# researchaccelerator-hub/distributed-crawler

Hardware: AMD Instinct MI355X
Metric: posts/sec (whole node) synthetic feed (higher is better)
Workload: dtype uint8; 1 GPU; model=telegram-crawl 1k-channels x 10k-posts per GPU (BASELINE config #2, weak-scaled), global_batch=1250000, seq_len=0, platform=telegram, parallelism=dp1, channels_per_gpu=1000, posts_per_channel=10000, chunk_posts=1250000, new_discoveries=998486, sink=pinned, pinned=True, max_comments_per_post=3

## Files before the change

### crawler_amd/ops/csrc/common.h

```cpp
#pragma once

#include <hip/hip_runtime.h>
#include <stdint.h>

#define WAVE 64
#define DEV __device__ __forceinline__

typedef unsigned int __attribute__((aligned(1))) u32_unal;
#ifndef CRAWL_NT_STORES
#define CRAWL_NT_STORES 0
#endif
DEV void nt_store_u32(unsigned char* p, unsigned v) {
#if CRAWL_NT_STORES
  __builtin_nontemporal_store(v, (u32_unal*)p);
#else
  __builtin_memcpy(p, &v, 4);
#endif
}
DEV void nt_store_u8(unsigned char* p, unsigned char v) {
#if CRAWL_NT_STORES
  __builtin_nontemporal_store(v, p);
#else
  *p = v;
#endif
}

namespace crawl {

DEV int lane_id() { return threadIdx.x & (WAVE - 1); }
DEV int wave_id() { return threadIdx.x >> 6; }


DEV bool is_ascii_letter(uint8_t c) {
  return (c >= 'a' && c <= 'z') || (c >= 'A' && c <= 'Z');
}
DEV bool is_word_char(uint8_t c) {
  return is_ascii_letter(c) || (c >= '0' && c <= '9') || c == '_';
}
DEV uint8_t to_lower(uint8_t c) {
  return (c >= 'A' && c <= 'Z') ? (c + 32) : c;
}

DEV int u16_units_of_byte(uint8_t b) {
  if (b < 0x80) return 1;
  if (b < 0xC0) return 0;
  if (b < 0xF0) return 1;
  return 2;
}

__device__ const uint8_t ESC_CLS[256] = {
    0x06, 0x06, 0x06, 0x06, 0x06, 0x06, 0x06, 0x06, 0x06, 0x02, 0x02, 0x06, 0x06, 0x02, 0x06, 0x06,
    0x06, 0x06, 0x06, 0x06, 0x06, 0x06, 0x06, 0x06, 0x06, 0x06, 0x06, 0x06, 0x06, 0x06, 0x06, 0x06,
    0x01, 0x01, 0x02, 0x01, 0x01, 0x01, 0x06, 0x01, 0x01, 0x01, 0x01, 0x01, 0x01, 0x01, 0x01, 0x01,
    0x01, 0x01, 0x01, 0x01, 0x01, 0x01, 0x01, 0x01, 0x01, 0x01, 0x01, 0x01, 0x06, 0x01, 0x06, 0x01,
    0x01, 0x01, 0x01, 0x01, 0x01, 0x01, 0x01, 0x01, 0x01, 0x01, 0x01, 0x01, 0x01, 0x01, 0x01, 0x01,
    0x01, 0x01, 0x01, 0x01, 0x01, 0x01, 0x01, 0x01, 0x01, 0x01, 0x01, 0x01, 0x02, 0x01, 0x01, 0x01,
    0x01, 0x01, 0x01, 0x01, 0x01, 0x01, 0x01, 0x01, 0x01, 0x01, 0x01, 0x01, 0x01, 0x01, 0x01, 0x01,
    0x01, 0x01, 0x01, 0x01, 0x01, 0x01, 0x01, 0x01, 0x01, 0x01, 0x01, 0x01, 0x01, 0x01, 0x01, 0x01,
    0xFF, 0x01, 0x01, 0x01, 0x01, 0x01, 0x01, 0x01, 0x01, 0x01, 0x01, 0x01, 0x01, 0x01, 0x01, 0x01,
    0x01, 0x01, 0x01, 0x01, 0x01, 0x01, 0x01, 0x01, 0x01, 0x01, 0x01, 0x01, 0x01, 0x01, 0x01, 0x01,
    0x01, 0x01, 0x01, 0x01, 0x01, 0x01, 0x01, 0x01, 0xFF, 0xFF, 0x01, 0x01, 0x01, 0x01, 0x01, 0x01,
    0x01, 0x01, 0x01, 0x01, 0x01, 0x01, 0x01, 0x01, 0x01, 0x01, 0x01, 0x01, 0x01, 0x01, 0x01, 0x01,
    0x01, 0x01, 0x01, 0x01, 0x01, 0x01, 0x01, 0x01, 0x01, 0x01, 0x01, 0x01, 0x01, 0x01, 0x01, 0x01,
    0x01, 0x01, 0x01, 0x01, 0x01, 0x01, 0x01, 0x01, 0x01, 0x01, 0x01, 0x01, 0x01, 0x01, 0x01, 0x01,
    0x01, 0x01, 0xFF, 0x01, 0x01, 0x01, 0x01, 0x01, 0x01, 0x01, 0x01, 0x01, 0x01, 0x01, 0x01, 0x01,
    0x01, 0x01, 0x01, 0x01, 0x01, 0x01, 0x01, 0x01, 0x01, 0x01, 0x01, 0x01, 0x01, 0x01, 0x01, 0x01,
};

DEV int escape_len_at(const uint8_t* s, int n, int p) {
  uint8_t c = s[p];
  uint8_t v = ESC_CLS[c];
  if (v != 0xFF) return v;
  if (c == 0xE2) {
    if (p + 2 < n && s[p + 1] == 0x80 &&
        (s[p + 2] == 0xA8 || s[p + 2] == 0xA9))
      return 6;
    return 1;
  }
  if (c == 0x80) {
    if (p >= 1 && s[p - 1] == 0xE2 && p + 1 < n &&
        (s[p + 1] == 0xA8 || s[p + 1] == 0xA9))
      return 0;
    return 1;
  }
  if (p >= 2 && s[p - 2] == 0xE2 && s[p - 1] == 0x80) return 0;
  return 1;
}

DEV const char* HEXD() { return "0123456789abcdef"; }

DEV int escape_write_at(const uint8_t* s, int n, int p, uint8_t* out) {
  uint8_t c = s[p];
  switch (c) {
    case '"':  out[0] = '\\'; out[1] = '"';  return 2;
    case '\\': out[0] = '\\'; out[1] = '\\'; return 2;
    case '\n': out[0] = '\\'; out[1] = 'n';  return 2;
    case '\r': out[0] = '\\'; out[1] = 'r';  return 2;
    case '\t': out[0] = '\\'; out[1] = 't';  return 2;
    default: break;
  }
  if (c < 0x20 || c == '<' || c == '>' || c == '&') {
    out[0] = '\\'; out[1] = 'u'; out[2] = '0'; out[3] = '0';
    out[4] = HEXD()[c >> 4]; out[5] = HEXD()[c & 15];
    return 6;
  }
  if (c == 0xE2 && p + 2 < n && s[p + 1] == 0x80 &&
      (s[p + 2] == 0xA8 || s[p + 2] == 0xA9)) {
    out[0] = '\\'; out[1] = 'u'; out[2] = '2'; out[3] = '0'; out[4] = '2';
    out[5] = (s[p + 2] == 0xA8) ? '8' : '9';
    return 6;
  }
  if (escape_len_at(s, n, p) == 0) return 0;
  out[0] = c;
  return 1;
}


DEV int wave_prefix_excl(int v) {
  int lane = lane_id();
  for (int d = 1; d < WAVE; d <<= 1) {
    int up = __shfl_up(v, d);
    if (lane >= d) v += up;
  }
  return __shfl_up(v, 1) * (lane > 0 ? 1 : 0);
}

DEV int wave_sum(int v) {
  for (int d = WAVE / 2; d > 0; d >>= 1) v += __shfl_down(v, d);
  return __shfl(v, 0);
}


DEV int u64_dec_len(uint64_t v) {
  if (v < 10ULL) return 1;
  if (v < 100ULL) return 2;
  if (v < 1000ULL) return 3;
  if (v < 10000ULL) return 4;
  if (v < 100000ULL) return 5;
  if (v < 1000000ULL) return 6;
  if (v < 10000000ULL) return 7;
  if (v < 100000000ULL) return 8;
  if (v < 1000000000ULL) return 9;
  if (v < 10000000000ULL) return 10;
  if (v < 100000000000ULL) return 11;
  if (v < 1000000000000ULL) return 12;
  if (v < 10000000000000ULL) return 13;
  if (v < 100000000000000ULL) return 14;
  if (v < 1000000000000000ULL) return 15;
  if (v < 10000000000000000ULL) return 16;
  if (v < 100000000000000000ULL) return 17;
  if (v < 1000000000000000000ULL) return 18;
  if (v < 10000000000000000000ULL) return 19;
  return 20;
}
DEV int i64_dec_len(int64_t v) {
  return (v < 0) ? 1 + u64_dec_len((uint64_t)(-v)) : u64_dec_len((uint64_t)v);
}

DEV void rfc3339_write(uint8_t* out, int cur, long long secs) {
  long long days = secs / 86400;
  long long rem = secs % 86400;
  if (rem < 0) { rem += 86400; days -= 1; }
  int hh = (int)(rem / 3600), mm = (int)((rem % 3600) / 60),
      ss = (int)(rem % 60);
  long long z = days + 719468;
  long long era = (z >= 0 ? z : z - 146096) / 146097;
  long long doe = z - era * 146097;
  long long yoe = (doe - doe / 1460 + doe / 36524 - doe / 146096) / 365;
  long long y = yoe + era * 400;
  long long doy = doe - (365 * yoe + yoe / 4 - yoe / 100);
  long long mp = (5 * doy + 2) / 153;
  long long d = doy - (153 * mp + 2) / 5 + 1;
  long long m = mp + (mp < 10 ? 3 : -9);
  y += (m <= 2);
  int yy = (int)y, mo = (int)m, dd = (int)d;
  auto pk = [](int a, int b, int c, int e) {
    return (unsigned)a | ((unsigned)b << 8) | ((unsigned)c << 16) |
           ((unsigned)e << 24);
  };
  unsigned w0 = pk('0' + (yy / 1000) % 10, '0' + (yy / 100) % 10,
                   '0' + (yy / 10) % 10, '0' + yy % 10);
  unsigned w1 = pk('-', '0' + mo / 10, '0' + mo % 10, '-');
  unsigned w2 = pk('0' + dd / 10, '0' + dd % 10, 'T', '0' + hh / 10);
  unsigned w3 = pk('0' + hh % 10, ':', '0' + mm / 10, '0' + mm % 10);
  unsigned w4 = pk(':', '0' + ss / 10, '0' + ss % 10, 'Z');
  int lane = lane_id();
  if (lane < 5) {
    unsigned v = w0;
    if (lane == 1) v = w1;
    else if (lane == 2) v = w2;
    else if (lane == 3) v = w3;
    else if (lane == 4) v = w4;
    nt_store_u32(out + cur + 4 * lane, v);
  }
}

#define LIT(e, s)                                              \
  do {                                                         \
    if ((int)sizeof(s) - 1 <= 4)                               \
      (e).template lit_small<(int)sizeof(s) - 1>(s);           \
    else                                                       \
      (e).raw((const unsigned char*)(s), (int)sizeof(s) - 1);  \
  } while (0)

template <bool W>
struct JsonEmit {
  uint8_t* out;
  int cur;
  const uint8_t* lds;

  DEV void lds_lit(int off, int n) {
    if (W) {
      const uint8_t* s = lds + off;
      int lane = lane_id();
      int nw = n >> 2;
      for (int k = lane; k < nw; k += WAVE) {
        unsigned w;
        __builtin_memcpy(&w, s + 4 * k, 4);
        nt_store_u32(out + cur + 4 * k, w);
      }
      for (int j = (nw << 2) + lane; j < n; j += WAVE)
        nt_store_u8(out + cur + j, s[j]);
    }
    cur += n;
  }

  template <int N, int M>
  DEV void lit_small(const char (&str)[M]) {
    if (W && lane_id() == 0) {
      if (N == 1) {
        out[cur] = (unsigned char)str[0];
      } else if (N == 2) {
        unsigned short v = (unsigned short)((unsigned char)str[0] |
                                            ((unsigned char)str[1] << 8));
        __builtin_memcpy(out + cur, &v, 2);
      } else {
        unsigned v = (unsigned)(unsigned char)str[0] |
                     ((unsigned)(unsigned char)str[1] << 8) |
                     ((N > 2 ? (unsigned)(unsigned char)str[2] : 0u) << 16) |
                     ((N > 3 ? (unsigned)(unsigned char)str[3] : 0u) << 24);
        if (N == 4)
          __builtin_memcpy(out + cur, &v, 4);
        else {
          __builtin_memcpy(out + cur, &v, 2);
          out[cur + 2] = (unsigned char)str[2];
        }
      }
    }
    cur += N;
  }

  DEV void raw(const uint8_t* s, int n) {
    if (W) {
      int lane = lane_id();
      int nw = n >> 2;
      for (int k = lane; k < nw; k += WAVE) {
        unsigned w;
        __builtin_memcpy(&w, s + 4 * k, 4);
        nt_store_u32(out + cur + 4 * k, w);
      }
      for (int j = (nw << 2) + lane; j < n; j += WAVE)
        nt_store_u8(out + cur + j, s[j]);
    }
    cur += n;
  }

  static DEV bool swar_special(unsigned w) {
    unsigned hz;
    unsigned nonascii = w & 0x80808080u;
    unsigned lt20 = (w - 0x20202020u) & ~w & 0x80808080u;
    if (lt20) return true;
    hz = ((w ^ 0x22222222u) - 0x01010101u) & ~(w ^ 0x22222222u);
    hz |= ((w ^ 0x5C5C5C5Cu) - 0x01010101u) & ~(w ^ 0x5C5C5C5Cu);
    hz |= ((w ^ 0x3C3C3C3Cu) - 0x01010101u) & ~(w ^ 0x3C3C3C3Cu);
    hz |= ((w ^ 0x3E3E3E3Eu) - 0x01010101u) & ~(w ^ 0x3E3E3E3Eu);
    hz |= ((w ^ 0x26262626u) - 0x01010101u) & ~(w ^ 0x26262626u);
    if (hz & 0x80808080u) return true;
    if (nonascii) {
      unsigned e2 = ((w ^ 0xE2E2E2E2u) - 0x01010101u) & ~(w ^ 0xE2E2E2E2u);
      if (e2 & 0x80808080u) return true;
    }
    return false;
  }

  DEV void esc(const uint8_t* s, int n) {
    int lane = lane_id();
    int start = 0;
    while (start < n) {
      if (start + 4 * WAVE <= n) {
        bool risk = (start >= 1 && s[start - 1] == 0xE2) ||
                    (start >= 2 && s[start - 2] == 0xE2 &&
                     s[start - 1] == 0x80);
        if (!risk) {
          unsigned w;
          __builtin_memcpy(&w, s + start + 4 * lane, 4);
          if (__ballot(swar_special(w)) == 0) {
            if (W)
              nt_store_u32(out + cur + 4 * lane, w);
            cur += 4 * WAVE;
            start += 4 * WAVE;
            continue;
          }
        }
      }
      esc_stripe(s, n, start, lane);
      start += WAVE;
    }
  }

  DEV void esc_stripe(const uint8_t* s, int n, int start, int lane) {
    {
      int p = start + lane;
      int span = n - start;
      if (span > WAVE) span = WAVE;
      int el = (p < n) ? escape_len_at(s, n, p) : 0;
      unsigned long long dirty = __ballot(p < n && el != 1);
      if (dirty == 0) {
        if (W && p < n) nt_store_u8(out + cur + p - start, s[p]);
        cur += span;
        return;
      }
      if (W) {
        int off = wave_prefix_excl(el);
        if (p < n && el > 0) {
          escape_write_at(s, n, p, out + cur + off);
        }
      }
      cur += wave_sum(el);
    }
  }

  DEV void u64(unsigned long long v) {
    static const unsigned long long POW10[20] = {
        1ULL, 10ULL, 100ULL, 1000ULL, 10000ULL, 100000ULL, 1000000ULL,
        10000000ULL, 100000000ULL, 1000000000ULL, 10000000000ULL,
        100000000000ULL, 1000000000000ULL, 10000000000000ULL,
        100000000000000ULL, 1000000000000000ULL, 10000000000000000ULL,
        100000000000000000ULL, 1000000000000000000ULL,
        10000000000000000000ULL};
    int n = u64_dec_len(v);
    if (W) {
      int lane = lane_id();
      if (lane < n) {
        unsigned d;
        if (v <= 0xFFFFFFFFULL)
          d = ((unsigned)v / (unsigned)POW10[lane]) % 10u;
        else
          d = (unsigned)((v / POW10[lane]) % 10ULL);
        nt_store_u8(out + cur + n - 1 - lane, (uint8_t)('0' + d));
      }
    }
    cur += n;
  }
  DEV void i64(long long v) {
    if (v < 0) { LIT(*this, "-"); u64((unsigned long long)(-v)); }
    else u64((unsigned long long)v);
  }

  DEV void rfc3339(long long secs) {
    if (W) rfc3339_write(out, cur, secs);
    cur += 20;
  }
};

DEV uint64_t fnv1a64(const uint8_t* s, int n) {
  uint64_t h = 1469598103934665603ULL;
  for (int i = 0; i < n; ++i) {
    h ^= s[i];
    h *= 1099511628211ULL;
  }
  return h;
}

}
```

### crawler_amd/ops/csrc/parse_encode.hip

```cpp

#include "common.h"
#include "tg_lits.h"

namespace crawl {

#define MAX_LINKS 8
#define TG_STAGE_BYTES 3968

struct BatchView {
  const long* __restrict__ chat_id;
  const long* __restrict__ msg_id;
  const long* __restrict__ text_off;
  const int* __restrict__ date;
  const int* __restrict__ content_type;
  const int* __restrict__ views;
  const int* __restrict__ forwards;
  const int* __restrict__ media_album_id;
  const int* __restrict__ channel_idx;
  const int* __restrict__ flags;
  const int* __restrict__ text_len;
  const int* __restrict__ aux_off;
  const int* __restrict__ aux_len;
  const int* __restrict__ ent_off;
  const int* __restrict__ ent_cnt;
  const int* __restrict__ react_off;
  const int* __restrict__ react_cnt;
  const int* __restrict__ com_off;
  const int* __restrict__ com_cnt;
  const int* __restrict__ poster_off;
  const int* __restrict__ poster_len;
  const unsigned char* __restrict__ pool;
  const int* __restrict__ entities;
  const int* __restrict__ react_emoji;
  const int* __restrict__ react_count;
  const int* __restrict__ com_text_off;
  const int* __restrict__ com_text_len;
  const int* __restrict__ com_handle_off;
  const int* __restrict__ com_handle_len;
  const int* __restrict__ com_views;
  const int* __restrict__ com_replies;
  const int* __restrict__ com_react_off;
  const int* __restrict__ com_react_cnt;
  const long* __restrict__ ch_chat_id;
  const int* __restrict__ ch_member;
  const int* __restrict__ ch_postcount;
  const int* __restrict__ ch_totalviews;
  const int* __restrict__ ch_user_off;
  const int* __restrict__ ch_user_len;
  const int* __restrict__ ch_title_off;
  const int* __restrict__ ch_title_len;
  const unsigned char* __restrict__ emoji_pool;
  const int* __restrict__ emoji_off;
  const int* __restrict__ emoji_len;
  const unsigned char* __restrict__ created_str;
  int created_len;
  const unsigned char* __restrict__ capture_str;
  int capture_len;
  int n;
  int skip_media;
  long min_post_date;
  const unsigned char* __restrict__ ctname_pool;
  const int* __restrict__ ctname_off;
  const int* __restrict__ ctname_len;
};

struct LinkOut {
  unsigned char* __restrict__ name;
  unsigned char* __restrict__ name_len;
  unsigned char* __restrict__ src;
  int* __restrict__ cnt;
  unsigned long long* __restrict__ hash;
};


DEV void utf16_to_bytes(const unsigned char* s, int n, int off16, int len16,
                        int* out_start, int* out_end) {
  int lane = lane_id();
  int run = 0;
  int start = -1, end = -1;
  const int t1 = off16, t2 = off16 + len16;
  for (int base = 0; base < n; base += WAVE) {
    int p = base + lane;
    int u = (p < n) ? u16_units_of_byte(s[p]) : 0;
    int pre = run + wave_prefix_excl(u);
    bool boundary = (p < n) && u > 0;
    unsigned long long m1 = __ballot(boundary && pre == t1);
    unsigned long long m2 = __ballot(boundary && pre == t2);
    if (start < 0 && m1) start = base + __ffsll(m1) - 1;
    if (end < 0 && m2) end = base + __ffsll(m2) - 1;
    run += wave_sum(u);
    if (end >= 0) break;
  }
  if (start < 0) { *out_start = 0; *out_end = 0; return; }
  *out_start = start;
  *out_end = (end >= 0) ? end : n;
}


DEV bool is_reserved_path(const unsigned char* name, int n) {
  const char* tbl[10] = {"joinchat", "addlist", "addstickers", "addtheme",
                         "setlanguage", "share", "proxy", "socks", "login",
                         "confirm"};
  const int lens[10] = {8, 7, 11, 8, 11, 5, 5, 5, 5, 7};
  for (int k = 0; k < 10; ++k) {
    if (lens[k] != n) continue;
    bool eq = true;
    for (int j = 0; j < n; ++j) eq &= (name[j] == (unsigned char)tbl[k][j]);
    if (eq) return true;
  }
  return false;
}

DEV int match_name_at(const unsigned char* s, int hi, int q,
                      unsigned char* name, bool* reserved) {
  *reserved = false;
  if (q >= hi || !is_ascii_letter(s[q])) return 0;
  int len = 0;
  while (len < 32 && q + len < hi && is_word_char(s[q + len])) ++len;
  if (len < 5) return 0;
  for (int j = 0; j < len; ++j) name[j] = to_lower(s[q + j]);
  *reserved = is_reserved_path(name, len);
  return len;
}

DEV int find_tme(const unsigned char* s, int from, int hi, int lane) {
  for (int base = from; base + 5 <= hi; base += WAVE) {
    int p = base + lane;
    bool m = (p + 5 <= hi) && s[p] == 't' && s[p + 1] == '.' &&
             s[p + 2] == 'm' && s[p + 3] == 'e' && s[p + 4] == '/';
    unsigned long long bal = __ballot(m);
    if (bal) return base + __ffsll(bal) - 1;
  }
  return -1;
}

DEV int find_username(const unsigned char* s, int lo, int hi, int lane,
                      unsigned char* name) {
  for (int base = lo; base < hi; base += WAVE) {
    int p = base + lane;
    bool m = false;
    if (p < hi && p + 5 <= hi && is_ascii_letter(s[p])) {
      m = is_word_char(s[p + 1]) && is_word_char(s[p + 2]) &&
          is_word_char(s[p + 3]) && is_word_char(s[p + 4]);
    }
    unsigned long long bal = __ballot(m);
    if (bal) {
      int q = base + __ffsll(bal) - 1;
      int len = 0;
      while (len < 32 && q + len < hi && is_word_char(s[q + len])) ++len;
      for (int j = 0; j < len; ++j) name[j] = to_lower(s[q + j]);
      return len;
    }
  }
  return 0;
}

struct LinkList {
  unsigned char* names;
  unsigned char* lens;
  unsigned char* srcs;
  unsigned long long* hashes;
  int cnt;

  DEV void add(const unsigned char* name, int len, int src, int lane) {
    for (int k = 0; k < cnt; ++k) {
      if (lens[k] != (unsigned char)len) continue;
      bool eq = true;
      for (int j = 0; j < len; ++j) eq &= (names[k * 32 + j] == name[j]);
      if (eq) return;
    }
    if (cnt >= MAX_LINKS) return;
    if (lane == 0) {
      for (int j = 0; j < len; ++j) names[cnt * 32 + j] = name[j];
      lens[cnt] = (unsigned char)len;
      srcs[cnt] = (unsigned char)src;
      hashes[cnt] = fnv1a64(name, len);
    }
    ++cnt;
  }
};

DEV void extract_links(const BatchView& B, int i, LinkList& L, int lane) {
  int ct = B.content_type[i];
  if (ct > 6) return;
  const unsigned char* text = B.pool + B.text_off[i];
  const int tn = B.text_len[i];
  unsigned char name[32];

  const int e0 = B.ent_off[i], ec = B.ent_cnt[i];
  for (int e = e0; e < e0 + ec; ++e) {
    const int* row = B.entities + (long)e * 5;
    int etype = row[0];
    if (etype == 1) {
      const unsigned char* url = B.pool + row[3];
      int un = row[4];
      for (int from = 0;;) {
        int p = find_tme(url, from, un, lane);
        if (p < 0) break;
        bool rsv;
        int len = match_name_at(url, un, p + 5, name, &rsv);
        if (len) {
          if (!rsv) L.add(name, len, 1, lane);
          break;
        }
        from = p + 1;
      }
    } else {
      int lo, hi;
      utf16_to_bytes(text, tn, row[1], row[2], &lo, &hi);
      if (!(lo < hi && hi <= tn)) continue;
      if (etype == 0) {
        int len = find_username(text, lo, hi, lane, name);
        if (len) L.add(name, len, 0, lane);
      } else {
        for (int from = lo;;) {
          int p = find_tme(text, from, hi, lane);
          if (p < 0) break;
          bool rsv;
          int len = match_name_at(text, hi, p + 5, name, &rsv);
          if (len) {
            if (!rsv) L.add(name, len, 2, lane);
            break;
          }
          from = p + 1;
        }
      }
    }
  }

  int cursor = 0;
  int from = 0;
  while (true) {
    int p = find_tme(text, from, tn, lane);
    if (p < 0) break;
    from = p + 1;
    if (p < cursor) continue;
    bool rsv;
    int len = match_name_at(text, tn, p + 5, name, &rsv);
    if (len) {
      if (!rsv) L.add(name, len, 3, lane);
      cursor = p + 5 + len;
      from = cursor;
    }
  }
}


template <bool W>
struct Emit : JsonEmit<W> {
  DEV void qesc(const unsigned char* s, int n) {
    LIT(*this, "\"");
    this->esc(s, n);
    LIT(*this, "\"");
  }
};

struct StagedTabs {
  const unsigned char* emoji_pool;
  const int* emoji_off;
  const int* emoji_len;
  const unsigned char* created;
  const unsigned char* capture;
  const unsigned char* ctname_pool;
  const int* ctname_off;
  const int* ctname_len;
};

template <bool W, bool STAGED>
DEV int emit_line(const BatchView& B, int i, unsigned char* out,
                  LinkList& L, const unsigned char* lds_lits,
                  unsigned char* lds_stage, const StagedTabs* T) {
  const int lane = lane_id();
  Emit<W> e{};
  e.out = out;
  e.cur = 0;
  e.lds = lds_lits;
  const int c = B.channel_idx[i];
  const unsigned char* user = B.pool + B.ch_user_off[c];
  const int user_n = B.ch_user_len[c];
  const unsigned char* title = B.pool + B.ch_title_off[c];
  const int title_n = B.ch_title_len[c];
  const long pub_id = B.msg_id[i] >> 20;
  const int ct = B.content_type[i];
  const int ncom = B.com_cnt[i];
  const bool has_user = user_n > 0;
  const long chat_id_v = B.chat_id[i];
  const int media_album = B.media_album_id[i];
  const int date_v = B.date[i];
  const int views_v = B.views[i];
  const int forwards_v = B.forwards[i];
  const int ch_member_v = B.ch_member[c];
  const int ch_postcount_v = B.ch_postcount[c];
  const int ch_totalviews_v = B.ch_totalviews[c];
  const int flags_v = B.flags[i];
  const int com0_v = B.com_off[i];
  const int react0_v = B.react_off[i];
  const int reactc_v = B.react_cnt[i];
  const int poster_off_v = B.poster_off[i];
  const int poster_len_v = B.poster_len[i];
  const int text_off_v = B.text_off[i];
  const int text_len_v = B.text_len[i];
  const int aux_off_v = B.aux_off[i];
  const int aux_len_v = B.aux_len[i];
  const int ctname_off_v = B.ctname_off[ct];
  const int ctname_len_v = B.ctname_len[ct];
  const unsigned char* desc_p;
  int desc_n;
  if (ct == 0 || ct == 1 || ct == 2 || ct == 4 || ct == 14) {
    desc_p = B.pool + text_off_v;
    desc_n = text_len_v;
  } else if (ct == 3 || ct == 9 || ct == 10 || ct == 11) {
    desc_p = B.pool + aux_off_v;
    desc_n = aux_len_v;
  } else {
    desc_p = nullptr;
    desc_n = 0;
  }
  const unsigned char* poster_p = B.pool + poster_off_v;
  const int* re_src = B.react_emoji + react0_v;
  const int* rcnt_src = B.react_count + react0_v;
  const unsigned char* lnames_src = L.names;
  const unsigned char* llens_src = L.lens;
  if (STAGED) {
    int stage_o = 0;
    auto staged = [&](const unsigned char* ptr,
                      int n) -> const unsigned char* {
      unsigned char* dst = lds_stage + stage_o;
      stage_o += n;
      for (int j = lane; j < n; j += WAVE) dst[j] = ptr[j];
      return dst;
    };
    user = staged(user, user_n);
    title = staged(title, title_n);
    poster_p = staged(poster_p, poster_len_v);
    desc_p = staged(desc_p, desc_n);
    lnames_src = staged(L.names, L.cnt * 32);
    llens_src = staged(L.lens, L.cnt);
    stage_o = (stage_o + 3) & ~3;
    int* s_re = (int*)(lds_stage + stage_o);
    stage_o += reactc_v * 4;
    int* s_rc = (int*)(lds_stage + stage_o);
    stage_o += reactc_v * 4;
    for (int j = lane; j < reactc_v; j += WAVE) {
      s_re[j] = B.react_emoji[react0_v + j];
      s_rc[j] = B.react_count[react0_v + j];
    }
    re_src = s_re;
    rcnt_src = s_rc;
  }
  const unsigned char* emoji_pool_s = STAGED ? T->emoji_pool : B.emoji_pool;
  const int* emoji_off_s = STAGED ? T->emoji_off : B.emoji_off;
  const int* emoji_len_s = STAGED ? T->emoji_len : B.emoji_len;
  const unsigned char* created_s = STAGED ? T->created : B.created_str;
  const unsigned char* capture_s = STAGED ? T->capture : B.capture_str;
  const unsigned char* ctpool_s = STAGED ? T->ctname_pool : B.ctname_pool;

  auto post_link = [&]() {
    if (!has_user) { LIT(e, "\"\""); return; }
    TGLIT(e, TGL_0);
    e.esc(user, user_n);
    LIT(e, "/");
    e.i64(pub_id);
    if (media_album != 0) TGLIT(e, TGL_1);
    LIT(e, "\"");
  };

  TGLIT(e, TGL_2);
  post_link();
  TGLIT(e, TGL_3);
  e.i64(chat_id_v);
  TGLIT(e, TGL_4);
  e.i64(pub_id);
  LIT(e, "-");
  e.esc(user, user_n);
  TGLIT(e, TGL_5);
  post_link();
  TGLIT(e, TGL_6);
  e.rfc3339(date_v);
  TGLIT(e, TGL_7);
  e.raw(created_s, B.created_len);
  TGLIT(e, TGL_8);
  e.i64(views_v);
  TGLIT(e, TGL_9);
  e.i64(views_v);
  TGLIT(e, TGL_10);
  e.i64(forwards_v);
  TGLIT(e, TGL_11);
  e.i64(ncom);
  TGLIT(e, TGL_12);
  e.qesc(title, title_n);
  TGLIT(e, TGL_13);
  e.i64(chat_id_v);
  TGLIT(e, TGL_14);
  e.qesc(title, title_n);
  TGLIT(e, TGL_15);
  e.i64(ch_member_v);
  TGLIT(e, TGL_16);
  e.i64(ch_postcount_v);
  TGLIT(e, TGL_17);
  e.i64(ch_totalviews_v);
  TGLIT(e, TGL_18);
  e.esc(user, user_n);
  TGLIT(e, TGL_19);
  e.esc(user, user_n);
  TGLIT(e, TGL_20);
  e.qesc(desc_p, desc_n);
  TGLIT(e, TGL_21);
  e.raw(ctpool_s + (STAGED ? T->ctname_off[ct] : ctname_off_v),
        STAGED ? T->ctname_len[ct] : ctname_len_v);
  TGLIT(e, TGL_22);
  e.i64(forwards_v);
  TGLIT(e, TGL_23);
  e.i64(ncom);
  TGLIT(e, TGL_17);
  e.i64(views_v);
  TGLIT(e, TGL_24);
  TGLIT(e, TGL_25);
  if ((ct == 3 || ct == 8) && (flags_v & 2)) {
    LIT(e, "AgAD");
    e.i64(pub_id);
    LIT(e, "v");
  }
  TGLIT(e, TGL_26);
  {
    const int c0 = com0_v;
    for (int k = 0; k < ncom; ++k) {
      if (k) LIT(e, ",");
      const int cc = c0 + k;
      TGLIT(e, TGL_27);
      e.qesc(B.pool + B.com_text_off[cc], B.com_text_len[cc]);
      TGLIT(e, TGL_28);
      const int r0 = B.com_react_off[cc], rc = B.com_react_cnt[cc];
      for (int r = 0; r < rc; ++r) {
        if (r) LIT(e, ",");
        int em = B.react_emoji[r0 + r];
        LIT(e, "\"");
        e.raw(emoji_pool_s + emoji_off_s[em], emoji_len_s[em]);
        LIT(e, "\":");
        e.i64(B.react_count[r0 + r]);
      }
      TGLIT(e, TGL_29);
      e.i64(B.com_views[cc]);
      TGLIT(e, TGL_30);
      e.i64(B.com_replies[cc]);
      TGLIT(e, TGL_31);
      e.qesc(B.pool + B.com_handle_off[cc], B.com_handle_len[cc]);
      LIT(e, "}");
    }
  }
  TGLIT(e, TGL_32);
  {
    const int rc = reactc_v;
    for (int r = 0; r < rc; ++r) {
      if (r) LIT(e, ",");
      int em = re_src[r];
      LIT(e, "\"");
      e.raw(emoji_pool_s + emoji_off_s[em], emoji_len_s[em]);
      LIT(e, "\":");
      e.i64(rcnt_src[r]);
    }
  }
  TGLIT(e, TGL_33);
  for (int k = 0; k < L.cnt; ++k) {
    if (k) LIT(e, ",");
    LIT(e, "\"");
    e.raw(lnames_src + k * 32, llens_src[k]);
    LIT(e, "\"");
  }
  TGLIT(e, TGL_34);
  e.raw(capture_s, B.capture_len);
  TGLIT(e, TGL_35);
  e.qesc(poster_p, poster_len_v);
  LIT(e, "}\n");
  return e.cur;
}


__global__ void __launch_bounds__(256, 6)
measure_extract_kernel(BatchView B, LinkOut LO, int* __restrict__ line_len) {
  __shared__ unsigned char s_lits[TG_POOL_BYTES];
  __shared__ unsigned char s_ln[4][MAX_LINKS * 32];
  __shared__ unsigned char s_ll[4][MAX_LINKS];
  __shared__ unsigned char s_ls[4][MAX_LINKS];
  __shared__ unsigned long long s_lh[4][MAX_LINKS];
  for (int t = threadIdx.x; t < TG_POOL_BYTES; t += blockDim.x)
    s_lits[t] = (unsigned char)tg_lit_pool.v[t];
  __syncthreads();
  const int lane = lane_id();
  const int wave = wave_id();
  const int waves_per_grid = gridDim.x * 4;
  for (int i = blockIdx.x * 4 + wave; i < B.n; i += waves_per_grid) {
    if ((long)B.date[i] < B.min_post_date) {
      if (lane == 0) { line_len[i] = 0; LO.cnt[i] = 0; }
      continue;
    }
    LinkList L{&s_ln[wave][0], &s_ll[wave][0], &s_ls[wave][0],
               &s_lh[wave][0], 0};
    extract_links(B, i, L, lane);
    int len = emit_line<false, false>(B, i, nullptr, L, s_lits,
                                     nullptr, nullptr);
    const int nb = L.cnt * 32;
    unsigned char* gname = LO.name + (size_t)i * MAX_LINKS * 32;
    for (int j = lane; j < nb; j += WAVE) gname[j] = s_ln[wave][j];
    if (lane < L.cnt) {
      LO.name_len[(size_t)i * MAX_LINKS + lane] = s_ll[wave][lane];
      LO.src[(size_t)i * MAX_LINKS + lane] = s_ls[wave][lane];
      LO.hash[(size_t)i * MAX_LINKS + lane] = s_lh[wave][lane];
    }
    if (lane == 0) {
      line_len[i] = len;
      LO.cnt[i] = L.cnt;
    }
  }
}

__global__ void __launch_bounds__(256, 4)
write_kernel(BatchView B, LinkOut LO, const long* __restrict__ line_off,
             const int* __restrict__ line_len, unsigned char* __restrict__ out) {
  __shared__ unsigned char s_lits[TG_POOL_BYTES];
  for (int t = threadIdx.x; t < TG_POOL_BYTES; t += blockDim.x)
    s_lits[t] = (unsigned char)tg_lit_pool.v[t];
  __syncthreads();
  const int lane = lane_id();
  const int wave = wave_id();
  const int waves_per_grid = gridDim.x * 4;
  for (int i = blockIdx.x * 4 + wave; i < B.n; i += waves_per_grid) {
    if (line_len[i] == 0) continue;
    LinkList L{LO.name + (size_t)i * MAX_LINKS * 32,
               LO.name_len + (size_t)i * MAX_LINKS,
               LO.src + (size_t)i * MAX_LINKS,
               LO.hash + (size_t)i * MAX_LINKS, LO.cnt[i]};
    emit_line<true, false>(B, i, out + line_off[i], L, s_lits, nullptr,
                           nullptr);
  }
}

#define TG_EMOJI_POOL_CAP 512
#define TG_EMOJI_CAP 64
#define TG_TS_CAP 64
#define TG_CTNAME_POOL_CAP 512
#define TG_CTNAME_CAP 32

__global__ void __launch_bounds__(256, 4)
write_staged_kernel(BatchView B, LinkOut LO, const long* __restrict__ line_off,
                    const int* __restrict__ line_len,
                    unsigned char* __restrict__ out,
                    int n_emoji, int emoji_pool_bytes,
                    int n_ctnames, int ctname_pool_bytes) {
  __shared__ unsigned char s_lits[TG_POOL_BYTES];
  __shared__ unsigned char s_stage[4][TG_STAGE_BYTES];
  __shared__ unsigned char s_emoji_pool[TG_EMOJI_POOL_CAP];
  __shared__ int s_emoji_off[TG_EMOJI_CAP];
  __shared__ int s_emoji_len[TG_EMOJI_CAP];
  __shared__ unsigned char s_created[TG_TS_CAP];
  __shared__ unsigned char s_capture[TG_TS_CAP];
  __shared__ unsigned char s_ctpool[TG_CTNAME_POOL_CAP];
  __shared__ int s_ctoff[TG_CTNAME_CAP];
  __shared__ int s_ctlen[TG_CTNAME_CAP];
  for (int t = threadIdx.x; t < TG_POOL_BYTES; t += blockDim.x)
    s_lits[t] = (unsigned char)tg_lit_pool.v[t];
  for (int t = threadIdx.x; t < emoji_pool_bytes; t += blockDim.x)
    s_emoji_pool[t] = B.emoji_pool[t];
  for (int t = threadIdx.x; t < n_emoji; t += blockDim.x) {
    s_emoji_off[t] = B.emoji_off[t];
    s_emoji_len[t] = B.emoji_len[t];
  }
  for (int t = threadIdx.x; t < B.created_len; t += blockDim.x)
    s_created[t] = B.created_str[t];
  for (int t = threadIdx.x; t < B.capture_len; t += blockDim.x)
    s_capture[t] = B.capture_str[t];
  for (int t = threadIdx.x; t < ctname_pool_bytes; t += blockDim.x)
    s_ctpool[t] = B.ctname_pool[t];
  for (int t = threadIdx.x; t < n_ctnames; t += blockDim.x) {
    s_ctoff[t] = B.ctname_off[t];
    s_ctlen[t] = B.ctname_len[t];
  }
  __syncthreads();
  StagedTabs T{s_emoji_pool, s_emoji_off, s_emoji_len, s_created,
               s_capture, s_ctpool, s_ctoff, s_ctlen};
  const int lane = lane_id();
  const int wave = wave_id();
  const int waves_per_grid = gridDim.x * 4;
  for (int i = blockIdx.x * 4 + wave; i < B.n; i += waves_per_grid) {
    if (line_len[i] == 0) continue;
    LinkList L{LO.name + (size_t)i * MAX_LINKS * 32,
               LO.name_len + (size_t)i * MAX_LINKS,
               LO.src + (size_t)i * MAX_LINKS,
               LO.hash + (size_t)i * MAX_LINKS, LO.cnt[i]};
    emit_line<true, true>(B, i, out + line_off[i], L, s_lits,
                          &s_stage[wave][0], &T);
  }
}


#define LDS_LINE_BYTES 3072

DEV void copy_line(const unsigned char* src, unsigned char* dst, int n,
                   int lane);

__global__ void __launch_bounds__(256)
write_lds_kernel(BatchView B, LinkOut LO, const long* __restrict__ line_off,
                 const int* __restrict__ line_len, unsigned char* __restrict__ out) {
  __shared__ unsigned char lbuf[4][LDS_LINE_BYTES];
  __shared__ unsigned char s_lits[TG_POOL_BYTES];
  for (int t = threadIdx.x; t < TG_POOL_BYTES; t += blockDim.x)
    s_lits[t] = (unsigned char)tg_lit_pool.v[t];
  __syncthreads();
  const int lane = lane_id();
  const int wave = wave_id();
  const int waves_per_grid = gridDim.x * 4;
  for (int i = blockIdx.x * 4 + wave; i < B.n; i += waves_per_grid) {
    const int len = line_len[i];
    if (len == 0) continue;
    LinkList L{LO.name + (size_t)i * MAX_LINKS * 32,
               LO.name_len + (size_t)i * MAX_LINKS,
               LO.src + (size_t)i * MAX_LINKS,
               LO.hash + (size_t)i * MAX_LINKS, LO.cnt[i]};
    if (len > LDS_LINE_BYTES) {
      emit_line<true, false>(B, i, out + line_off[i], L, s_lits,
                             nullptr, nullptr);
      continue;
    }
    emit_line<true, false>(B, i, &lbuf[wave][0], L, s_lits, nullptr,
                           nullptr);
    copy_line(&lbuf[wave][0], out + line_off[i], len, lane);
  }
}


__global__ void __launch_bounds__(256)
write_scratch_kernel(BatchView B, LinkOut LO, unsigned char* __restrict__ scratch,
                     long stride, int* __restrict__ line_len, int* __restrict__ overflow) {
  __shared__ unsigned char s_lits[TG_POOL_BYTES];
  for (int t = threadIdx.x; t < TG_POOL_BYTES; t += blockDim.x)
    s_lits[t] = (unsigned char)tg_lit_pool.v[t];
  __syncthreads();
  const int lane = lane_id();
  const int wave = wave_id();
  const int waves_per_grid = gridDim.x * 4;
  for (int i = blockIdx.x * 4 + wave; i < B.n; i += waves_per_grid) {
    if ((long)B.date[i] < B.min_post_date) {
      if (lane == 0) { line_len[i] = 0; LO.cnt[i] = 0; }
      continue;
    }
    LinkList L{LO.name + (size_t)i * MAX_LINKS * 32,
               LO.name_len + (size_t)i * MAX_LINKS,
               LO.src + (size_t)i * MAX_LINKS,
               LO.hash + (size_t)i * MAX_LINKS, 0};
    extract_links(B, i, L, lane);
    int len = emit_line<true, false>(B, i, scratch + (size_t)i * stride, L,
                                     s_lits, nullptr, nullptr);
    if (lane == 0) {
      line_len[i] = len;
      LO.cnt[i] = L.cnt;
      if (len > stride) atomicMax(overflow, len);
    }
  }
}

DEV void copy_line(const unsigned char* src, unsigned char* dst, int n,
                   int lane) {
  int h = (int)((4 - ((unsigned long)(size_t)dst & 3)) & 3);
  if (h > n) h = n;
  if (lane == 0)
    for (int j = 0; j < h; ++j) dst[j] = src[j];
  const unsigned char* s = src + h;
  unsigned char* d = dst + h;
  int rem = n - h;
  int nw = rem >> 2;
  int sh = (int)((unsigned long)(size_t)s & 3);
  const unsigned int* sw = (const unsigned int*)(s - sh);
  for (int k = lane; k < nw; k += WAVE) {
    unsigned int w0 = sw[k];
    unsigned int v;
    if (sh) {
      unsigned int w1 = sw[k + 1];
      v = (unsigned int)((((unsigned long long)w1 << 32) | w0) >> (8 * sh));
    } else {
      v = w0;
    }
    ((unsigned int*)d)[k] = v;
  }
  if (lane == 0)
    for (int j = h + (nw << 2); j < n; ++j) dst[j] = src[j];
}

__global__ void __launch_bounds__(256)
compact_kernel(const unsigned char* scratch, long stride,
               const long* line_off, const int* line_len,
               unsigned char* out, int n) {
  const int lane = lane_id();
  const int wave = wave_id();
  const int waves_per_grid = gridDim.x * 4;
  for (int i = blockIdx.x * 4 + wave; i < n; i += waves_per_grid) {
    int len = line_len[i];
    if (len == 0) continue;
    copy_line(scratch + (size_t)i * stride, out + line_off[i], len, lane);
  }
}

}


namespace crawl {

static BatchView make_view(void** p, const long* s) {
  BatchView B;
  int k = 0;
  B.chat_id = (const long*)p[k++];
  B.msg_id = (const long*)p[k++];
  B.text_off = (const long*)p[k++];
  B.date = (const int*)p[k++];
  B.content_type = (const int*)p[k++];
  B.views = (const int*)p[k++];
  B.forwards = (const int*)p[k++];
  B.media_album_id = (const int*)p[k++];
  B.channel_idx = (const int*)p[k++];
  B.flags = (const int*)p[k++];
  B.text_len = (const int*)p[k++];
  B.aux_off = (const int*)p[k++];
  B.aux_len = (const int*)p[k++];
  B.ent_off = (const int*)p[k++];
  B.ent_cnt = (const int*)p[k++];
  B.react_off = (const int*)p[k++];
  B.react_cnt = (const int*)p[k++];
  B.com_off = (const int*)p[k++];
  B.com_cnt = (const int*)p[k++];
  B.poster_off = (const int*)p[k++];
  B.poster_len = (const int*)p[k++];
  B.pool = (const unsigned char*)p[k++];
  B.entities = (const int*)p[k++];
  B.react_emoji = (const int*)p[k++];
  B.react_count = (const int*)p[k++];
  B.com_text_off = (const int*)p[k++];
  B.com_text_len = (const int*)p[k++];
  B.com_handle_off = (const int*)p[k++];
  B.com_handle_len = (const int*)p[k++];
  B.com_views = (const int*)p[k++];
  B.com_replies = (const int*)p[k++];
  B.com_react_off = (const int*)p[k++];
  B.com_react_cnt = (const int*)p[k++];
  B.ch_chat_id = (const long*)p[k++];
  B.ch_member = (const int*)p[k++];
  B.ch_postcount = (const int*)p[k++];
  B.ch_totalviews = (const int*)p[k++];
  B.ch_user_off = (const int*)p[k++];
  B.ch_user_len = (const int*)p[k++];
  B.ch_title_off = (const int*)p[k++];
  B.ch_title_len = (const int*)p[k++];
  B.emoji_pool = (const unsigned char*)p[k++];
  B.emoji_off = (const int*)p[k++];
  B.emoji_len = (const int*)p[k++];
  B.created_str = (const unsigned char*)p[k++];
  B.capture_str = (const unsigned char*)p[k++];
  B.ctname_pool = (const unsigned char*)p[k++];
  B.ctname_off = (const int*)p[k++];
  B.ctname_len = (const int*)p[k++];
  B.n = (int)s[0];
  B.skip_media = (int)s[1];
  B.min_post_date = s[2];
  B.created_len = (int)s[3];
  B.capture_len = (int)s[4];
  return B;
}

static LinkOut make_links(void** p) {
  LinkOut L;
  L.name = (unsigned char*)p[0];
  L.name_len = (unsigned char*)p[1];
  L.src = (unsigned char*)p[2];
  L.cnt = (int*)p[3];
  L.hash = (unsigned long long*)p[4];
  return L;
}

}

extern "C" {

int crawl_batch_ptr_count() { return 49; }

int crawl_measure_extract(void** batch_ptrs, const long* scalars,
                          void** link_ptrs, void* line_len, int grid,
                          void* stream) {
  crawl::BatchView B = crawl::make_view(batch_ptrs, scalars);
  crawl::LinkOut LO = crawl::make_links(link_ptrs);
  hipLaunchKernelGGL(crawl::measure_extract_kernel, dim3(grid), dim3(256), 0,
                     (hipStream_t)stream, B, LO, (int*)line_len);
  return (int)hipGetLastError();
}

int crawl_write(void** batch_ptrs, const long* scalars, void** link_ptrs,
                const void* line_off, const void* line_len, void* out,
                int grid, void* stream) {
  crawl::BatchView B = crawl::make_view(batch_ptrs, scalars);
  crawl::LinkOut LO = crawl::make_links(link_ptrs);
  hipLaunchKernelGGL(crawl::write_kernel, dim3(grid), dim3(256), 0,
                     (hipStream_t)stream, B, LO, (const long*)line_off,
                     (const int*)line_len, (unsigned char*)out);
  return (int)hipGetLastError();
}

int crawl_write_staged(void** batch_ptrs, const long* scalars,
                       void** link_ptrs, const void* line_off,
                       const void* line_len, void* out,
                       int n_emoji, int emoji_pool_bytes,
                       int n_ctnames, int ctname_pool_bytes,
                       int grid, void* stream) {
  crawl::BatchView B = crawl::make_view(batch_ptrs, scalars);
  crawl::LinkOut LO = crawl::make_links(link_ptrs);
  hipLaunchKernelGGL(crawl::write_staged_kernel, dim3(grid), dim3(256), 0,
                     (hipStream_t)stream, B, LO, (const long*)line_off,
                     (const int*)line_len, (unsigned char*)out,
                     n_emoji, emoji_pool_bytes, n_ctnames,
                     ctname_pool_bytes);
  return (int)hipGetLastError();
}

int crawl_stage_budget() { return TG_STAGE_BYTES; }

int crawl_write_scratch(void** batch_ptrs, const long* scalars,
                        void** link_ptrs, void* scratch, long stride,
                        void* line_len, void* overflow, int grid,
                        void* stream) {
  crawl::BatchView B = crawl::make_view(batch_ptrs, scalars);
  crawl::LinkOut LO = crawl::make_links(link_ptrs);
  hipLaunchKernelGGL(crawl::write_scratch_kernel, dim3(grid), dim3(256), 0,
                     (hipStream_t)stream, B, LO, (unsigned char*)scratch,
                     stride, (int*)line_len, (int*)overflow);
  return (int)hipGetLastError();
}

int crawl_write_lds(void** batch_ptrs, const long* scalars, void** link_ptrs,
                    const void* line_off, const void* line_len, void* out,
                    int grid, void* stream) {
  crawl::BatchView B = crawl::make_view(batch_ptrs, scalars);
  crawl::LinkOut LO = crawl::make_links(link_ptrs);
  hipLaunchKernelGGL(crawl::write_lds_kernel, dim3(grid), dim3(256), 0,
                     (hipStream_t)stream, B, LO, (const long*)line_off,
                     (const int*)line_len, (unsigned char*)out);
  return (int)hipGetLastError();
}

int crawl_compact(const void* scratch, long stride, const void* line_off,
                  const void* line_len, void* out, int n, int grid,
                  void* stream) {
  hipLaunchKernelGGL(crawl::compact_kernel, dim3(grid), dim3(256), 0,
                     (hipStream_t)stream, (const unsigned char*)scratch,
                     stride, (const long*)line_off, (const int*)line_len,
                     (unsigned char*)out, n);
  return (int)hipGetLastError();
}

}
```

Before: 27.91 million posts/s.

## Precompute decimal fields, 32-bit date and int formatting, reuse escape lengths, scalarize wave ids

Each numeric field is formatted once into per-lane digit characters using 32-bit multiply-high division, and the result is reused at every place the field appears. Repeated escapes of user, title and nick skip the measuring pass when the line is not being written. Dates and counts now go through 32-bit arithmetic, wave ids are read as uniform scalars, and the link name buffer moves from per-lane private memory to LDS written by lane 0. The goal is to cut 64-bit division, repeated formatting work and scratch-memory pressure in the JSON emit kernels. In exchange, formatted digits stay live in registers across the whole line, and the int32 paths assume those fields fit in 32 bits.

After: 27.97 million posts/s, median of 6. No clear change (+0.2%).

```diff
diff --git a/crawler_amd/ops/csrc/common.h b/crawler_amd/ops/csrc/common.h
--- a/crawler_amd/ops/csrc/common.h
+++ b/crawler_amd/ops/csrc/common.h
@@ -29,6 +29,9 @@
 
 DEV int lane_id() { return threadIdx.x & (WAVE - 1); }
 DEV int wave_id() { return threadIdx.x >> 6; }
+DEV int wave_id_uniform() {
+  return __builtin_amdgcn_readfirstlane((int)(threadIdx.x >> 6));
+}
 
 
 DEV bool is_ascii_letter(uint8_t c) {
@@ -157,6 +160,73 @@
   return (v < 0) ? 1 + u64_dec_len((uint64_t)(-v)) : u64_dec_len((uint64_t)v);
 }
 
+DEV unsigned sgpr_opaque(unsigned x) {
+  unsigned r = __builtin_amdgcn_readfirstlane(x);
+  asm("" : "+s"(r));
+  return r;
+}
+
+DEV int u32_dec_len(uint32_t v) {
+  if (v < 10u) return 1;
+  if (v < 100u) return 2;
+  if (v < 1000u) return 3;
+  if (v < 10000u) return 4;
+  if (v < 100000u) return 5;
+  if (v < 1000000u) return 6;
+  if (v < 10000000u) return 7;
+  if (v < 100000000u) return 8;
+  if (v < 1000000000u) return 9;
+  return 10;
+}
+
+struct Pow10x32 { unsigned d, m; };
+__device__ const Pow10x32 POW10_32[10] = {
+    {1u, 4294967295u},   {10u, 429496729u},   {100u, 42949672u},
+    {1000u, 4294967u},   {10000u, 429496u},   {100000u, 42949u},
+    {1000000u, 4294u},   {10000000u, 429u},   {100000000u, 42u},
+    {1000000000u, 4u}};
+
+DEV void rfc3339_store(uint8_t* out, int cur, unsigned yy, unsigned mo,
+                       unsigned dd, unsigned hh, unsigned mm, unsigned ss) {
+  auto pk = [](unsigned a, unsigned b, unsigned c, unsigned e) {
+    return a | (b << 8) | (c << 16) | (e << 24);
+  };
+  unsigned w0 = pk('0' + (yy / 1000) % 10, '0' + (yy / 100) % 10,
+                   '0' + (yy / 10) % 10, '0' + yy % 10);
+  unsigned w1 = pk('-', '0' + mo / 10, '0' + mo % 10, '-');
+  unsigned w2 = pk('0' + dd / 10, '0' + dd % 10, 'T', '0' + hh / 10);
+  unsigned w3 = pk('0' + hh % 10, ':', '0' + mm / 10, '0' + mm % 10);
+  unsigned w4 = pk(':', '0' + ss / 10, '0' + ss % 10, 'Z');
+  int lane = lane_id();
+  if (lane < 5) {
+    unsigned v = w0;
+    if (lane == 1) v = w1;
+    else if (lane == 2) v = w2;
+    else if (lane == 3) v = w3;
+    else if (lane == 4) v = w4;
+    nt_store_u32(out + cur + 4 * lane, v);
+  }
+}
+
+DEV void rfc3339_write32(uint8_t* out, int cur, int secs) {
+  int days = secs / 86400;
+  int rem = secs - days * 86400;
+  if (rem < 0) { rem += 86400; days -= 1; }
+  unsigned r = (unsigned)rem;
+  unsigned hh = r / 3600u, mm = (r % 3600u) / 60u, ss = r % 60u;
+  unsigned z = (unsigned)(days + 719468);
+  unsigned era = z / 146097u;
+  unsigned doe = z - era * 146097u;
+  unsigned yoe = (doe - doe / 1460u + doe / 36524u - doe / 146096u) / 365u;
+  unsigned y = yoe + era * 400u;
+  unsigned doy = doe - (365u * yoe + yoe / 4u - yoe / 100u);
+  unsigned mp = (5u * doy + 2u) / 153u;
+  unsigned d = doy - (153u * mp + 2u) / 5u + 1u;
+  unsigned m = mp < 10u ? mp + 3u : mp - 9u;
+  y += (m <= 2u);
+  rfc3339_store(out, cur, y, m, d, hh, mm, ss);
+}
+
 DEV void rfc3339_write(uint8_t* out, int cur, long long secs) {
   long long days = secs / 86400;
   long long rem = secs % 86400;
@@ -173,26 +243,8 @@
   long long d = doy - (153 * mp + 2) / 5 + 1;
   long long m = mp + (mp < 10 ? 3 : -9);
   y += (m <= 2);
-  int yy = (int)y, mo = (int)m, dd = (int)d;
-  auto pk = [](int a, int b, int c, int e) {
-    return (unsigned)a | ((unsigned)b << 8) | ((unsigned)c << 16) |
-           ((unsigned)e << 24);
-  };
-  unsigned w0 = pk('0' + (yy / 1000) % 10, '0' + (yy / 100) % 10,
-                   '0' + (yy / 10) % 10, '0' + yy % 10);
-  unsigned w1 = pk('-', '0' + mo / 10, '0' + mo % 10, '-');
-  unsigned w2 = pk('0' + dd / 10, '0' + dd % 10, 'T', '0' + hh / 10);
-  unsigned w3 = pk('0' + hh % 10, ':', '0' + mm / 10, '0' + mm % 10);
-  unsigned w4 = pk(':', '0' + ss / 10, '0' + ss % 10, 'Z');
-  int lane = lane_id();
-  if (lane < 5) {
-    unsigned v = w0;
-    if (lane == 1) v = w1;
-    else if (lane == 2) v = w2;
-    else if (lane == 3) v = w3;
-    else if (lane == 4) v = w4;
-    nt_store_u32(out + cur + 4 * lane, v);
-  }
+  rfc3339_store(out, cur, (unsigned)y, (unsigned)m, (unsigned)d,
+                (unsigned)hh, (unsigned)mm, (unsigned)ss);
 }
 
 #define LIT(e, s)                                              \
@@ -208,11 +260,11 @@
   uint8_t* out;
   int cur;
   const uint8_t* lds;
+  int lane = lane_id();
 
   DEV void lds_lit(int off, int n) {
     if (W) {
       const uint8_t* s = lds + off;
-      int lane = lane_id();
       int nw = n >> 2;
       for (int k = lane; k < nw; k += WAVE) {
         unsigned w;
@@ -227,7 +279,7 @@
 
   template <int N, int M>
   DEV void lit_small(const char (&str)[M]) {
-    if (W && lane_id() == 0) {
+    if (W && lane == 0) {
       if (N == 1) {
         out[cur] = (unsigned char)str[0];
       } else if (N == 2) {
@@ -252,7 +304,6 @@
 
   DEV void raw(const uint8_t* s, int n) {
     if (W) {
-      int lane = lane_id();
       int nw = n >> 2;
       for (int k = lane; k < nw; k += WAVE) {
         unsigned w;
@@ -284,7 +335,6 @@
   }
 
   DEV void esc(const uint8_t* s, int n) {
-    int lane = lane_id();
     int start = 0;
     while (start < n) {
       if (start + 4 * WAVE <= n) {
@@ -340,7 +390,6 @@
         10000000000000000000ULL};
     int n = u64_dec_len(v);
     if (W) {
-      int lane = lane_id();
       if (lane < n) {
         unsigned d;
         if (v <= 0xFFFFFFFFULL)
@@ -357,8 +406,80 @@
     else u64((unsigned long long)v);
   }
 
+  struct Dec {
+    unsigned ch;
+    int n;
+  };
+
+  static DEV unsigned digit32(unsigned a, int j) {
+    const Pow10x32 p = POW10_32[j];
+    unsigned q = __umulhi(a, p.m);
+    if (a - q * p.d >= p.d) ++q;
+    return q % 10u;
+  }
+
+  DEV Dec dec_u32(unsigned a, bool neg) {
+    const int nd = u32_dec_len(a);
+    Dec x;
+    x.n = nd + (neg ? 1 : 0);
+    x.ch = '-';
+    if (W) {
+      if (lane < nd) x.ch = '0' + digit32(a, lane);
+    }
+    return x;
+  }
+
+  DEV Dec dec32(int v) {
+    const bool neg = v < 0;
+    return dec_u32(neg ? 0u - (unsigned)v : (unsigned)v, neg);
+  }
+
+  DEV Dec dec64(long long v) {
+    const bool neg = v < 0;
+    const unsigned long long a =
+        neg ? 0ULL - (unsigned long long)v : (unsigned long long)v;
+    if (sgpr_opaque((unsigned)(a >> 32)) == 0)
+      return dec_u32(sgpr_opaque((unsigned)a), neg);
+    const unsigned long long q = a / 1000000000ULL;
+    const unsigned lo = sgpr_opaque((unsigned)(a - q * 1000000000ULL));
+    const unsigned hi = sgpr_opaque((unsigned)(q / 1000000000ULL));
+    const unsigned mid =
+        sgpr_opaque((unsigned)(q - (unsigned long long)hi * 1000000000ULL));
+    const int nd = hi ? 18 + u32_dec_len(hi) : 9 + u32_dec_len(mid);
+    Dec x;
+    x.n = nd + (neg ? 1 : 0);
+    x.ch = '-';
+    if (W) {
+      if (lane < nd) {
+        unsigned c = lane < 9 ? lo : (lane < 18 ? mid : hi);
+        int j = lane < 9 ? lane : (lane < 18 ? lane - 9 : lane - 18);
+        x.ch = '0' + digit32(c, j);
+      }
+    }
+    return x;
+  }
+
+  DEV void put(const Dec& x) {
+    if (W) {
+      if (lane < x.n)
+        nt_store_u8(out + cur + x.n - 1 - lane, (uint8_t)x.ch);
+    }
+    cur += x.n;
+  }
+
+  DEV void i32(int v) { put(dec32(v)); }
+
+  DEV void esc_again(const uint8_t* s, int n, int el) {
+    if (W) esc(s, n);
+    else cur += el;
+  }
+
   DEV void rfc3339(long long secs) {
     if (W) rfc3339_write(out, cur, secs);
+    cur += 20;
+  }
+  DEV void rfc3339_i32(int secs) {
+    if (W) rfc3339_write32(out, cur, secs);
     cur += 20;
   }
 };
diff --git a/crawler_amd/ops/csrc/parse_encode.hip b/crawler_amd/ops/csrc/parse_encode.hip
--- a/crawler_amd/ops/csrc/parse_encode.hip
+++ b/crawler_amd/ops/csrc/parse_encode.hip
@@ -118,7 +118,8 @@
   int len = 0;
   while (len < 32 && q + len < hi && is_word_char(s[q + len])) ++len;
   if (len < 5) return 0;
-  for (int j = 0; j < len; ++j) name[j] = to_lower(s[q + j]);
+  if (lane_id() == 0)
+    for (int j = 0; j < len; ++j) name[j] = to_lower(s[q + j]);
   *reserved = is_reserved_path(name, len);
   return len;
 }
@@ -148,7 +149,8 @@
       int q = base + __ffsll(bal) - 1;
       int len = 0;
       while (len < 32 && q + len < hi && is_word_char(s[q + len])) ++len;
-      for (int j = 0; j < len; ++j) name[j] = to_lower(s[q + j]);
+      if (lane == 0)
+        for (int j = 0; j < len; ++j) name[j] = to_lower(s[q + j]);
       return len;
     }
   }
@@ -180,12 +182,12 @@
   }
 };
 
-DEV void extract_links(const BatchView& B, int i, LinkList& L, int lane) {
+DEV void extract_links(const BatchView& B, int i, LinkList& L, int lane,
+                       unsigned char* name) {
   int ct = B.content_type[i];
   if (ct > 6) return;
   const unsigned char* text = B.pool + B.text_off[i];
   const int tn = B.text_len[i];
-  unsigned char name[32];
 
   const int e0 = B.ent_off[i], ec = B.ent_cnt[i];
   for (int e = e0; e < e0 + ec; ++e) {
@@ -270,8 +272,13 @@
 DEV int emit_line(const BatchView& B, int i, unsigned char* out,
                   LinkList& L, const unsigned char* lds_lits,
                   unsigned char* lds_stage, const StagedTabs* T) {
-  const int lane = lane_id();
+  int lane = lane_id();
+  if (W) {
+    asm volatile("" : "+v"(lane));
+    lane &= WAVE - 1;
+  }
   Emit<W> e{};
+  e.lane = lane;
   e.out = out;
   e.cur = 0;
   e.lds = lds_lits;
@@ -355,70 +362,101 @@
   const unsigned char* capture_s = STAGED ? T->capture : B.capture_str;
   const unsigned char* ctpool_s = STAGED ? T->ctname_pool : B.ctname_pool;
 
-  auto post_link = [&]() {
+  const auto pub_id_d = e.dec64(pub_id);
+  const auto chat_id_d = e.dec64(chat_id_v);
+  const auto views_d = e.dec32(views_v);
+  const auto forwards_d = e.dec32(forwards_v);
+  const auto ncom_d = e.dec32(ncom);
+  int user_el = 0;
+  auto post_link = [&](bool first) {
     if (!has_user) { LIT(e, "\"\""); return; }
     TGLIT(e, TGL_0);
-    e.esc(user, user_n);
+    if (first) {
+      const int c0 = e.cur;
+      e.esc(user, user_n);
+      user_el = e.cur - c0;
+    } else {
+      e.esc_again(user, user_n, user_el);
+    }
     LIT(e, "/");
-    e.i64(pub_id);
+    e.put(pub_id_d);
     if (media_album != 0) TGLIT(e, TGL_1);
     LIT(e, "\"");
   };
 
+  const unsigned char* nick_p = has_user ? user : title;
+  const int nick_n = has_user ? user_n : title_n;
+  int nick_title_el = 0;
+  if (!has_user) {
+    Emit<false> m{};
+    m.cur = 0;
+    m.esc(title, title_n);
+    nick_title_el = m.cur;
+  }
+  auto nick = [&]() {
+    e.esc_again(nick_p, nick_n, has_user ? user_el : nick_title_el);
+  };
+
   TGLIT(e, TGL_2);
-  post_link();
+  post_link(true);
   TGLIT(e, TGL_3);
-  e.i64(chat_id_v);
+  e.put(chat_id_d);
   TGLIT(e, TGL_4);
-  e.i64(pub_id);
+  e.put(pub_id_d);
   LIT(e, "-");
-  e.esc(user, user_n);
+  nick();
   TGLIT(e, TGL_5);
-  post_link();
+  post_link(false);
   TGLIT(e, TGL_6);
-  e.rfc3339(date_v);
+  e.rfc3339_i32(date_v);
   TGLIT(e, TGL_7);
   e.raw(created_s, B.created_len);
   TGLIT(e, TGL_8);
-  e.i64(views_v);
+  e.put(views_d);
   TGLIT(e, TGL_9);
-  e.i64(views_v);
+  e.put(views_d);
   TGLIT(e, TGL_10);
-  e.i64(forwards_v);
+  e.put(forwards_d);
   TGLIT(e, TGL_11);
-  e.i64(ncom);
+  e.put(ncom_d);
   TGLIT(e, TGL_12);
-  e.qesc(title, title_n);
+  LIT(e, "\"");
+  const int title_c0 = e.cur;
+  e.esc(title, title_n);
+  const int title_el = e.cur - title_c0;
+  LIT(e, "\"");
   TGLIT(e, TGL_13);
-  e.i64(chat_id_v);
+  e.put(chat_id_d);
   TGLIT(e, TGL_14);
-  e.qesc(title, title_n);
+  LIT(e, "\"");
+  e.esc_again(title, title_n, title_el);
+  LIT(e, "\"");
   TGLIT(e, TGL_15);
-  e.i64(ch_member_v);
+  e.i32(ch_member_v);
   TGLIT(e, TGL_16);
-  e.i64(ch_postcount_v);
+  e.i32(ch_postcount_v);
   TGLIT(e, TGL_17);
-  e.i64(ch_totalviews_v);
+  e.i32(ch_totalviews_v);
   TGLIT(e, TGL_18);
-  e.esc(user, user_n);
+  nick();
   TGLIT(e, TGL_19);
-  e.esc(user, user_n);
+  nick();
   TGLIT(e, TGL_20);
   e.qesc(desc_p, desc_n);
   TGLIT(e, TGL_21);
   e.raw(ctpool_s + (STAGED ? T->ctname_off[ct] : ctname_off_v),
         STAGED ? T->ctname_len[ct] : ctname_len_v);
   TGLIT(e, TGL_22);
-  e.i64(forwards_v);
+  e.put(forwards_d);
   TGLIT(e, TGL_23);
-  e.i64(ncom);
+  e.put(ncom_d);
   TGLIT(e, TGL_17);
-  e.i64(views_v);
+  e.put(views_d);
   TGLIT(e, TGL_24);
   TGLIT(e, TGL_25);
   if ((ct == 3 || ct == 8) && (flags_v & 2)) {
     LIT(e, "AgAD");
-    e.i64(pub_id);
+    e.put(pub_id_d);
     LIT(e, "v");
   }
   TGLIT(e, TGL_26);
@@ -437,12 +475,12 @@
         LIT(e, "\"");
         e.raw(emoji_pool_s + emoji_off_s[em], emoji_len_s[em]);
         LIT(e, "\":");
-        e.i64(B.react_count[r0 + r]);
+        e.i32(B.react_count[r0 + r]);
       }
       TGLIT(e, TGL_29);
-      e.i64(B.com_views[cc]);
+      e.i32(B.com_views[cc]);
       TGLIT(e, TGL_30);
-      e.i64(B.com_replies[cc]);
+      e.i32(B.com_replies[cc]);
       TGLIT(e, TGL_31);
       e.qesc(B.pool + B.com_handle_off[cc], B.com_handle_len[cc]);
       LIT(e, "}");
@@ -457,7 +495,7 @@
       LIT(e, "\"");
       e.raw(emoji_pool_s + emoji_off_s[em], emoji_len_s[em]);
       LIT(e, "\":");
-      e.i64(rcnt_src[r]);
+      e.i32(rcnt_src[r]);
     }
   }
   TGLIT(e, TGL_33);
@@ -483,11 +521,12 @@
   __shared__ unsigned char s_ll[4][MAX_LINKS];
   __shared__ unsigned char s_ls[4][MAX_LINKS];
   __shared__ unsigned long long s_lh[4][MAX_LINKS];
+  __shared__ unsigned char s_name[4][32];
   for (int t = threadIdx.x; t < TG_POOL_BYTES; t += blockDim.x)
     s_lits[t] = (unsigned char)tg_lit_pool.v[t];
   __syncthreads();
   const int lane = lane_id();
-  const int wave = wave_id();
+  const int wave = wave_id_uniform();
   const int waves_per_grid = gridDim.x * 4;
   for (int i = blockIdx.x * 4 + wave; i < B.n; i += waves_per_grid) {
     if ((long)B.date[i] < B.min_post_date) {
@@ -496,7 +535,7 @@
     }
     LinkList L{&s_ln[wave][0], &s_ll[wave][0], &s_ls[wave][0],
                &s_lh[wave][0], 0};
-    extract_links(B, i, L, lane);
+    extract_links(B, i, L, lane, &s_name[wave][0]);
     int len = emit_line<false, false>(B, i, nullptr, L, s_lits,
                                      nullptr, nullptr);
     const int nb = L.cnt * 32;
@@ -522,7 +561,7 @@
     s_lits[t] = (unsigned char)tg_lit_pool.v[t];
   __syncthreads();
   const int lane = lane_id();
-  const int wave = wave_id();
+  const int wave = wave_id_uniform();
   const int waves_per_grid = gridDim.x * 4;
   for (int i = blockIdx.x * 4 + wave; i < B.n; i += waves_per_grid) {
     if (line_len[i] == 0) continue;
@@ -579,7 +618,7 @@
   StagedTabs T{s_emoji_pool, s_emoji_off, s_emoji_len, s_created,
                s_capture, s_ctpool, s_ctoff, s_ctlen};
   const int lane = lane_id();
-  const int wave = wave_id();
+  const int wave = wave_id_uniform();
   const int waves_per_grid = gridDim.x * 4;
   for (int i = blockIdx.x * 4 + wave; i < B.n; i += waves_per_grid) {
     if (line_len[i] == 0) continue;
@@ -607,7 +646,7 @@
     s_lits[t] = (unsigned char)tg_lit_pool.v[t];
   __syncthreads();
   const int lane = lane_id();
-  const int wave = wave_id();
+  const int wave = wave_id_uniform();
   const int waves_per_grid = gridDim.x * 4;
   for (int i = blockIdx.x * 4 + wave; i < B.n; i += waves_per_grid) {
     const int len = line_len[i];
@@ -632,11 +671,12 @@
 write_scratch_kernel(BatchView B, LinkOut LO, unsigned char* __restrict__ scratch,
                      long stride, int* __restrict__ line_len, int* __restrict__ overflow) {
   __shared__ unsigned char s_lits[TG_POOL_BYTES];
+  __shared__ unsigned char s_name[4][32];
   for (int t = threadIdx.x; t < TG_POOL_BYTES; t += blockDim.x)
     s_lits[t] = (unsigned char)tg_lit_pool.v[t];
   __syncthreads();
   const int lane = lane_id();
-  const int wave = wave_id();
+  const int wave = wave_id_uniform();
   const int waves_per_grid = gridDim.x * 4;
   for (int i = blockIdx.x * 4 + wave; i < B.n; i += waves_per_grid) {
     if ((long)B.date[i] < B.min_post_date) {
@@ -647,7 +687,7 @@
                LO.name_len + (size_t)i * MAX_LINKS,
                LO.src + (size_t)i * MAX_LINKS,
                LO.hash + (size_t)i * MAX_LINKS, 0};
-    extract_links(B, i, L, lane);
+    extract_links(B, i, L, lane, &s_name[wave][0]);
     int len = emit_line<true, false>(B, i, scratch + (size_t)i * stride, L,
                                      s_lits, nullptr, nullptr);
     if (lane == 0) {
@@ -690,7 +730,7 @@
                const long* line_off, const int* line_len,
                unsigned char* out, int n) {
   const int lane = lane_id();
-  const int wave = wave_id();
+  const int wave = wave_id_uniform();
   const int waves_per_grid = gridDim.x * 4;
   for (int i = blockIdx.x * 4 + wave; i < n; i += waves_per_grid) {
     int len = line_len[i];
```
